# tlkvstepan/PracticalDeepStereo_NIPS2018

Measured on AMD Instinct MI355X. Metric: stereo pairs/sec, 960x540 D=192, Matching+Regularization+SubpixelMap hot path, higher is better.
Workload: dtype f32; 1 GPU; configs[1]: 960x540 pair padded to 576x960, D=192 (48 matching planes, 96 cost planes), batch 1, eval mode, random-init weights seed 0; parallelism=single GPU, launch=eager, whole pairs round-robin over 3 HIP streams

## Files before the change

### practicaldeepstereo_nips2018_amd/csrc/upsample_estimator.hip

```cpp
#include <type_traits>

#include "common.hpp"

namespace pds {

namespace {

constexpr int TR = 4, TC = 32;
constexpr int HR = TR + 2, HC = TC + 2;
constexpr int NPOS = HR * HC;
constexpr int HS = 48;
constexpr int TILE_CH = HR * HS;
constexpr int POS = (NPOS + 63) / 64;
typedef float f32x16 __attribute__((ext_vector_type(16)));
typedef float f32x2 __attribute__((ext_vector_type(2)));

struct FusedArgs {
    const float* __restrict__ in;
    const float* __restrict__ scale;
    const float* __restrict__ shift;
    const float* __restrict__ w;
    const float* __restrict__ bias;
    float* __restrict__ disp;
    float* __restrict__ cost;
    int D, Hi, Wi;
    int lo, hi;
    float step;
    int crop_top, crop_left;
    float* __restrict__ conf;
};

}

constexpr int UHALF = 128;
constexpr int UPOS = (NPOS + UHALF - 1) / UHALF;
constexpr int EO = HC / 2;

template <bool CAND>
__device__ __forceinline__ void estimator_update2(float v, float h1, float h2, int k, int km1, int km2, float& best, int& bi,
                                                  float& bp0, float& bp1, float& bn0, float& bn1) {
    unsigned long long m0, m1, mu;
    if constexpr (CAND) {
        asm volatile(
            "v_cmp_eq_u32_e64 %[m0], %[bi], %[km1]\n\t"
            "v_cmp_eq_u32_e64 %[m1], %[bi], %[km2]\n\t"
            "v_cmp_gt_f32_e64 %[mu], %[v], %[best]\n\t"
            "v_cndmask_b32_e64 %[bn0], %[bn0], %[v], %[m0]\n\t"
            "v_cndmask_b32_e64 %[bn1], %[bn1], %[v], %[m1]\n\t"
            "s_nop 0\n\t"
            "v_cndmask_b32_e64 %[best], %[best], %[v], %[mu]\n\t"
            "v_cndmask_b32_e64 %[bi], %[bi], %[kv], %[mu]\n\t"
            "v_cndmask_b32_e64 %[bp0], %[bp0], %[h1], %[mu]\n\t"
            "v_cndmask_b32_e64 %[bp1], %[bp1], %[h2], %[mu]"
            : [m0] "=&s"(m0), [m1] "=&s"(m1), [mu] "=&s"(mu), [best] "+v"(best), [bi] "+v"(bi), [bp0] "+v"(bp0),
              [bp1] "+v"(bp1), [bn0] "+v"(bn0), [bn1] "+v"(bn1)
            : [v] "v"(v), [h1] "v"(h1), [h2] "v"(h2), [kv] "v"(k), [km1] "s"(km1), [km2] "s"(km2));
    } else {
        asm volatile(
            "v_cmp_eq_u32_e64 %[m0], %[bi], %[km1]\n\t"
            "v_cmp_eq_u32_e64 %[m1], %[bi], %[km2]\n\t"
            "s_nop 1\n\t"
            "v_cndmask_b32_e64 %[bn0], %[bn0], %[v], %[m0]\n\t"
            "v_cndmask_b32_e64 %[bn1], %[bn1], %[v], %[m1]"
            : [m0] "=&s"(m0), [m1] "=&s"(m1), [bn0] "+v"(bn0), [bn1] "+v"(bn1)
            : [v] "v"(v), [bi] "v"(bi), [km1] "s"(km1), [km2] "s"(km2));
    }
}

template <int CIN, int T, bool WRITE_COST, int PY, int DS, bool CONF, bool MIRROR>
__device__ __forceinline__ void upsample_sweep(const FusedArgs& A, float (*tile)[CIN][TILE_CH], float* merge, const int part) {
    constexpr int R = 3 + T;
    constexpr int U = (R % 2 == 0) ? R : 2 * R;
    const int tid = threadIdx.x & (UHALF - 1);
    const int lane = tid & 63;
    const int r = lane >> 4, cp = lane & 15;
    const int i0 = blockIdx.y * TR, j0 = blockIdx.x * TC;
    const int b = blockIdx.z;
    const size_t plane = (size_t)A.Hi * A.Wi;
    const size_t cstride = (size_t)A.D * plane;
    const unsigned plane_bytes = (unsigned)(plane * sizeof(float)), cbytes = (unsigned)(cstride * sizeof(float));
    const __amdgpu_buffer_rsrc_t rsrc = __builtin_amdgcn_make_buffer_rsrc(
        const_cast<float*>(A.in + (size_t)b * CIN * cstride), 0, (int)(CIN * cstride * sizeof(float)), 0x00020000);

    const int per = (A.D + DS - 1) / DS;
    const int lo = DS == 1 ? 0 : part * per, hi = DS == 1 ? A.D : min(A.D, lo + per);
    const int pb = DS == 1 ? 0 : max(lo - T - 1, 0);
    const int pe = WRITE_COST ? A.D : hi + T;
    int nsteps = pe - pb + 1;
    if (DS > 1) {
#pragma unroll
        for (int q = 0; q < DS; ++q) {
            const int lq = q * per, hq = min(A.D, lq + per);
            nsteps = max(nsteps, hq + T - max(lq - T - 1, 0) + 1);
        }
    }

    unsigned goff[UPOS];
    int loff[UPOS];
    bool inside[UPOS];
#pragma unroll
    for (int k = 0; k < UPOS; ++k) {
        const int p = min(tid + k * UHALF, NPOS - 1);
        const int rr = p / HC, cc = p % HC;
        const int y = i0 - 1 + rr, x = j0 - 1 + cc;
        inside[k] = y >= 0 && y < A.Hi && x >= 0 && x < A.Wi;
#ifdef PDS_UPS_NOHALO
        goff[k] = (unsigned)(min(max(y, i0), min(i0 + TR, A.Hi) - 1) * A.Wi + min(max(x, j0), min(j0 + TC, A.Wi) - 1)) * 4u;
#else
        goff[k] = inside[k] ? (unsigned)(y * A.Wi + x) * 4u : 0x80000000u;
#endif
        loff[k] = rr * HS + (cc & 1) * EO + (cc >> 1);
    }
    float sc[CIN], shv[CIN][UPOS];
#pragma unroll
    for (int c = 0; c < CIN; ++c) {
        sc[c] = A.scale ? A.scale[b * CIN + c] : 1.f;
        const float sh = A.scale ? A.shift[b * CIN + c] : 0.f;
#pragma unroll
        for (int k = 0; k < UPOS; ++k) shv[c][k] = inside[k] ? sh : 0.f;
    }
    const float bias = A.bias ? A.bias[0] : 0.f;

    float st[2][CIN][UPOS];
#ifdef PDS_UPS_NOLDSWRITE
    float sink = 0.f;
#define PDS_UPS_STORE(dst_, v_) sink += (v_);
#else
#define PDS_UPS_STORE(dst_, v_) dst_ = (v_);
#endif
#define PDS_FETCHP(set_, p_)                                                       \
    _Pragma("unroll") for (int c = 0; c < CIN; ++c) _Pragma("unroll") for (int k = 0; k < UPOS; ++k) \
        st[set_][c][k] = __builtin_bit_cast(float, __builtin_amdgcn_raw_buffer_load_b32(               \
            rsrc, goff[k], (unsigned)(p_) * plane_bytes + c * cbytes, 0));
#define PDS_STASHP(set_, buf_)                                                     \
    _Pragma("unroll") for (int c = 0; c < CIN; ++c) _Pragma("unroll") for (int k = 0; k < UPOS; ++k) \
        PDS_UPS_STORE(tile[buf_][c][loff[k]], fmaf(sc[c], st[set_][c][k], shv[c][k]))

#ifdef PDS_UPS_TIMING
    long long tm[4] = {0, 0, 0, 0};
#endif
    float best[4], bprev[4][T], bnext[4][T], mass[4];
    int bi[4];
#pragma unroll
    for (int o = 0; o < 4; ++o) {
        best[o] = -INFINITY;
        if constexpr (CONF) mass[o] = 0.f;
        bi[o] = lo;
#pragma unroll
        for (int t = 0; t < T; ++t) bprev[o][t] = bnext[o][t] = -INFINITY;
    }
    f32x2 ring[R][2];
#pragma unroll
    for (int q = 0; q < R; ++q) ring[q][0] = ring[q][1] = f32x2{bias, bias};

    PDS_FETCHP(1, pb)
    if (pb + 1 < A.D) PDS_FETCHP(0, pb + 1)
    PDS_STASHP(1, 0)
    __syncthreads();

    const int lbase = r * HS + cp;
    auto plane_step = [&](auto jc, const int step) __attribute__((always_inline)) {
        constexpr int J = decltype(jc)::value;
        constexpr int SF = J % R, S0 = (J + 1) % R, S1 = (J + 2) % R;
        constexpr int SX = J & 1, SY = SX ^ 1;
        const int p = pb + step;
        ring[S1][0] = ring[S1][1] = f32x2{bias, bias};
#ifdef PDS_UPS_TIMING
        const long long t0 = __builtin_readcyclecounter();
        long long t1 = t0, t2 = t0;
#endif
        if (p < A.D && p <= pe) {
#ifndef PDS_UPS_NOSTAGE
            if (p + 2 < A.D && p + 2 <= pe) PDS_FETCHP(SY, p + 2)
#endif
#pragma nounroll
            for (int c2 = 0; c2 < CIN; c2 += 2) {
                f32x2 r02[2][2], r13[2][2];
#pragma unroll
                for (int cc = 0; cc < 2; ++cc)
#pragma unroll
                    for (int a = 0; a < 2; ++a) {
                        const int vr = (a == 0) ? 1 : (PY == 0 ? 0 : 2);
                        const float* row = &tile[SX][c2 + cc][lbase + vr * HS];
#ifdef PDS_UPS_NOLDSREAD
                        r02[cc][a] = f32x2{sc[cc], shv[a][0]};
                        r13[cc][a] = f32x2{shv[cc][1], sc[a]};
                        continue;
#endif
                        r02[cc][a] = f32x2{row[0], row[1]};
                        r13[cc][a] = f32x2{row[EO], row[EO + 1]};
                    }
                f32x16 wk[3];
#ifdef PDS_UPS_NOSLOAD
// ... 97 lines not shown
                        bprev[o][t] = up ? ring[SP][o >> 1][o & 1] : bprev[o][t];
                    }
                }
            }
        }
#ifdef PDS_UPS_TIMING
        tm[3] += __builtin_readcyclecounter() - t3;
#endif
    };
#ifdef PDS_UPS_TIMING
    const long long t_begin = __builtin_readcyclecounter();
#endif
    for (int base = 0; base < nsteps; base += U) {
#define PDS_STEP(J_) if (base + J_ < nsteps) plane_step(std::integral_constant<int, J_>{}, base + J_);
        PDS_STEP(0) PDS_STEP(1) PDS_STEP(2) PDS_STEP(3)
        if constexpr (U > 4) { PDS_STEP(4) PDS_STEP(5) PDS_STEP(6) PDS_STEP(7) PDS_STEP(8) PDS_STEP(9) }
        if constexpr (U > 10) { PDS_STEP(10) PDS_STEP(11) PDS_STEP(12) PDS_STEP(13) }
#undef PDS_STEP
    }
    static_assert(U == 4 || U == 10 || U == 14, "unrolled groups of T = 1, 2, 4");
#ifdef PDS_UPS_TIMING
    {
        const int wgl = blockIdx.y * gridDim.x + blockIdx.x;
        unsigned hwid, xcc;
        asm volatile("s_getreg_b32 %0, hwreg(HW_REG_HW_ID)" : "=s"(hwid));
        asm volatile("s_getreg_b32 %0, hwreg(HW_REG_XCC_ID)" : "=s"(xcc));
        if (lane == 0 && (wgl % 97) == 0)
            printf("[ups] wg %d part %d py %d xcc %u hwid %08x: start %lld total %lld | channels %lld stash %lld barrier %lld estimator %lld (%d steps)\n",
                   wgl, part, PY, xcc & 15, hwid, t_begin, (long long)__builtin_readcyclecounter() - t_begin, tm[0], tm[1], tm[2], tm[3], nsteps);
    }
#endif
#undef PDS_FETCHP
#undef PDS_STASHP
#undef PDS_UPS_STORE
#ifdef PDS_UPS_NOLDSWRITE
    if (sink == 12345.f) best[0] = sink;
#endif

    if (WRITE_COST) return;
    if (DS > 1) {
        constexpr int ITEMS = 4 * (2 + 2 * T) + (CONF ? 4 : 0);
        float* mine = merge + ((size_t)(part > 0 ? part - 1 : 0) * 2 + PY) * ITEMS * 64 + lane;
        if (part > 0) {
#pragma unroll
            for (int o = 0; o < 4; ++o) {
                mine[(o * (2 + 2 * T) + 0) * 64] = best[o];
                mine[(o * (2 + 2 * T) + 1) * 64] = __int_as_float(bi[o]);
#pragma unroll
                for (int t = 0; t < T; ++t) {
                    mine[(o * (2 + 2 * T) + 2 + t) * 64] = bprev[o][t];
                    mine[(o * (2 + 2 * T) + 2 + T + t) * 64] = bnext[o][t];
                }
                if constexpr (CONF) mine[(4 * (2 + 2 * T) + o) * 64] = mass[o];
            }
        }
        __syncthreads();
        if (part > 0) return;
#pragma unroll
        for (int q = 1; q < DS; ++q) {
            const float* theirs = merge + ((size_t)(q - 1) * 2 + PY) * ITEMS * 64 + lane;
#pragma unroll
            for (int o = 0; o < 4; ++o) {
                const float other = theirs[(o * (2 + 2 * T) + 0) * 64];
                if constexpr (CONF) {
                    const float m = fmaxf(best[o], other);
                    mass[o] = mass[o] * expf(best[o] - m) + theirs[(4 * (2 + 2 * T) + o) * 64] * expf(other - m);
                }
                const bool up = other > best[o];
                best[o] = up ? other : best[o];
                bi[o] = up ? __float_as_int(theirs[(o * (2 + 2 * T) + 1) * 64]) : bi[o];
// ... 48 lines not shown
                float* cdst = A.conf + ((size_t)b * Hc + row) * Wc;
                if (vec) {
                    *reinterpret_cast<float4*>(cdst + mcol) = make_float4(cres[3], cres[2], cres[1], cres[0]);
                } else {
#pragma unroll
                    for (int o = 0; o < 4; ++o)
                        if (o < valid && col + o >= 0) cdst[Wc - 1 - col - o] = cres[o];
                }
            }
        } else if (row >= 0) {
            float* dst = A.disp + ((size_t)b * Hc + row) * Wc + col;
            const int valid = (j + 1 < A.Wi) ? 4 : 2;
            if (valid == 4 && col >= 0 && ((A.crop_left | Wc) & 3) == 0) {
                *reinterpret_cast<float4*>(dst) = make_float4(res[0], res[1], res[2], res[3]);
            } else {
#pragma unroll
                for (int o = 0; o < 4; ++o)
                    if (o < valid && col + o >= 0) dst[o] = res[o];
            }
            if constexpr (CONF) {
                float* cdst = A.conf + ((size_t)b * Hc + row) * Wc + col;
                if (valid == 4 && col >= 0 && ((A.crop_left | Wc) & 3) == 0) {
                    *reinterpret_cast<float4*>(cdst) = make_float4(cres[0], cres[1], cres[2], cres[3]);
                } else {
#pragma unroll
                    for (int o = 0; o < 4; ++o)
                        if (o < valid && col + o >= 0) cdst[o] = cres[o];
                }
            }
        }
    }
}

template <int CIN, int T, bool WRITE_COST, int DS, bool CONF = false, bool MIRROR = false>
__global__ __launch_bounds__(UHALF * DS, (DS == 2 && T <= 2) ? ((CONF && T == 2) ? 4 : 5) : 1) void upsample_full_subpixel_kernel(const FusedArgs A) {
    constexpr int TILE = 2 * CIN * TILE_CH, MERGE = (DS - 1) * 2 * (4 * (2 + 2 * T) + (CONF ? 4 : 0)) * 64;
    constexpr int FLOATS = DS * TILE > MERGE ? DS * TILE : MERGE;
    __shared__ __attribute__((aligned(16))) float lds[FLOATS];
    const int wave = __builtin_amdgcn_readfirstlane(threadIdx.x >> 6);
    const int part = wave >> 1;
    float (*tile)[CIN][TILE_CH] = reinterpret_cast<float (*)[CIN][TILE_CH]>(lds + part * TILE);
    if ((wave & 1) == 0)
        upsample_sweep<CIN, T, WRITE_COST, 0, DS, CONF, MIRROR>(A, tile, lds, part);
    else
        upsample_sweep<CIN, T, WRITE_COST, 1, DS, CONF, MIRROR>(A, tile, lds, part);
}

__global__ void upsample_weight_pairs_kernel(const float* __restrict__ w, float* __restrict__ w_pairs, int cin) {
    const int e = blockIdx.x * blockDim.x + threadIdx.x;
    if (e >= cin * 48) return;
    const int j = e & 3, a = (e >> 2) & 1, kd = (e >> 3) % 3, c = (e / 24) % cin, py = e / (24 * cin);
    const int kh = a == 0 ? 1 + py : 3 - 3 * py;
    w_pairs[e] = w[((c * 3 + kd) * 4 + kh) * 4 + ((j + 1) & 3)];
}

int launch_upsample_weight_pairs(const float* w, float* w_pairs, int cin, hipStream_t s) {
    const int total = cin * 48;
    hipLaunchKernelGGL(upsample_weight_pairs_kernel, dim3((total + 255) / 256), dim3(256), 0, s, w, w_pairs, cin);
    return check_launch("upsample_weight_pairs");
}

bool upsample_estimator_supported(int cin, int lo, int hi) {
    const int t = (-lo > hi) ? -lo : hi;
    return cin == 4 && t >= 1 && t <= 4;
}

int launch_upsample_estimator(const float* in, const float* scale, const float* shift, const float* w,
                              const float* bias, float* disp, int batch, int cin, int d, int hi_, int wi, int lo,
                              int hi, int step, int crop_top, int crop_left, hipStream_t s, float* conf, bool mirror) {
    FusedArgs A;
    A.conf = conf;
    A.crop_top = crop_top;
    A.crop_left = crop_left;
    A.in = in;
    A.scale = scale;
    A.shift = shift;
    A.w = w;
    A.bias = bias;
    A.disp = disp;
    A.D = d;
    A.Hi = hi_;
    A.Wi = wi;
    A.lo = lo;
    A.hi = hi;
    A.step = (float)step;
    dim3 grid((wi + TC - 1) / TC, (hi_ + TR - 1) / TR, batch);
    const int t = (-lo > hi) ? -lo : hi;
    if (cin != 4) return set_error(-1, "upsample_estimator: unsupported channel count %d", cin);
    A.cost = nullptr;
    if (mirror) {
        if (conf) {
            if (t <= 1)
                hipLaunchKernelGGL((upsample_full_subpixel_kernel<4, 1, false, 2, true, true>), grid, dim3(2 * UHALF), 0, s,
                                   A);
            else if (t <= 2)
                hipLaunchKernelGGL((upsample_full_subpixel_kernel<4, 2, false, 2, true, true>), grid, dim3(2 * UHALF), 0, s,
                                   A);
            else
                hipLaunchKernelGGL((upsample_full_subpixel_kernel<4, 4, false, 2, true, true>), grid, dim3(2 * UHALF), 0, s,
                                   A);
            return check_launch("upsample_full_subpixel_confidence_mirrored");
        }
        if (t <= 1)
            hipLaunchKernelGGL((upsample_full_subpixel_kernel<4, 1, false, 2, false, true>), grid, dim3(2 * UHALF), 0, s, A);
        else if (t <= 2)
            hipLaunchKernelGGL((upsample_full_subpixel_kernel<4, 2, false, 2, false, true>), grid, dim3(2 * UHALF), 0, s, A);
        else
            hipLaunchKernelGGL((upsample_full_subpixel_kernel<4, 4, false, 2, false, true>), grid, dim3(2 * UHALF), 0, s, A);
        return check_launch("upsample_full_subpixel_mirrored");
    }
    if (conf) {
        if (t <= 1)
            hipLaunchKernelGGL((upsample_full_subpixel_kernel<4, 1, false, 2, true>), grid, dim3(2 * UHALF), 0, s, A);
        else if (t <= 2)
            hipLaunchKernelGGL((upsample_full_subpixel_kernel<4, 2, false, 2, true>), grid, dim3(2 * UHALF), 0, s, A);
        else
            hipLaunchKernelGGL((upsample_full_subpixel_kernel<4, 4, false, 2, true>), grid, dim3(2 * UHALF), 0, s, A);
        return check_launch("upsample_full_subpixel_confidence");
    }
    if (t <= 1)
        hipLaunchKernelGGL((upsample_full_subpixel_kernel<4, 1, false, 2>), grid, dim3(2 * UHALF), 0, s, A);
    else if (t <= 2)
        hipLaunchKernelGGL((upsample_full_subpixel_kernel<4, 2, false, 2>), grid, dim3(2 * UHALF), 0, s, A);
    else
        hipLaunchKernelGGL((upsample_full_subpixel_kernel<4, 4, false, 2>), grid, dim3(2 * UHALF), 0, s, A);
    return check_launch("upsample_full_subpixel");
}

bool upsample_full_valu_supported(int cin) { return cin == 4; }

int launch_upsample_full(const float* in, const float* scale, const float* shift, const float* w, const float* bias,
                         float* cost, int batch, int cin, int d, int hi_, int wi, hipStream_t s) {
    if (cin != 4) return set_error(-1, "upsample_full: unsupported channel count %d", cin);
    FusedArgs A;
    A.in = in;
    A.scale = scale;
    A.shift = shift;
    A.w = w;
    A.bias = bias;
    A.disp = nullptr;
    A.cost = cost;
    A.D = d;
    A.Hi = hi_;
    A.Wi = wi;
    A.lo = 0;
    A.hi = 0;
    A.step = 0.f;
    A.crop_top = A.crop_left = 0;
    A.conf = nullptr;
    dim3 grid((wi + TC - 1) / TC, (hi_ + TR - 1) / TR, batch);
    hipLaunchKernelGGL((upsample_full_subpixel_kernel<4, 1, true, 1>), grid, dim3(UHALF), 0, s, A);
    return check_launch("upsample_full");
}

}
```

### practicaldeepstereo_nips2018_amd/csrc/conv2d_t8.hip

```cpp
#include <atomic>
#include <type_traits>

#include "common.hpp"

namespace pds {

namespace {

constexpr int C2_THREADS = 256;
constexpr int C2_CIN = 64, C2_COUT = 8, C2_KC = 4, C2_CHUNKS = C2_CIN / C2_KC;
constexpr int C2_TY = 16, C2_NB = 2, C2_TX = 16 * C2_NB, C2_RP = C2_TY / 8;
constexpr int C2_YT = C2_TY + 2, C2_XT = C2_TX + 2, C2_RS = 36;
constexpr int C2_PART = C2_YT * C2_RS * 8;
constexpr int C2_BUF = 2 * C2_PART;
constexpr int C2_AFRAGS = C2_CHUNKS * 3 * 2;
constexpr int C2_ABYTES = C2_AFRAGS * 64 * 8;
constexpr int C2_NPOS = C2_YT * C2_XT;
constexpr int C2_POS = (C2_NPOS + C2_THREADS - 1) / C2_THREADS;
static_assert(C2_RS >= C2_XT, "LDS row");
typedef float f32x4 __attribute__((ext_vector_type(4)));
typedef _Float16 f16x4 __attribute__((ext_vector_type(4)));

struct C2Args {
    Src a, b;
// ... 279 lines not shown
        if (c == C2_CHUNKS - 1) {
            const int out_base = (int)((size_t)Pcur.nb * C2_COUT * cstride * sizeof(float));
#pragma unroll
            for (int p = 0; p < C2_RP; ++p)
#pragma unroll
                for (int r = 0; r < 4; ++r) {
                    const int h = r >> 1, y = Pcur.y0 + 2 * (C2_RP * wave + p) + (r & 1);
                    const int row_bytes = __builtin_amdgcn_readfirstlane(
                        out_base + (int)(((size_t)Pcur.d * A.H + min(y, A.H - 1)) * A.W + Pcur.x0) * (int)sizeof(float));
#pragma unroll
                    for (int j = 0; j < C2_NB; ++j) {
                        float t = acc[p][j][r] * SC.unscale;
                        if (A.lrelu) t = fmaxf(t, t * kLeakySlope);
                        const bool ok = y < A.H && Pcur.x0 + 16 * j + n16 < A.W;
                        __builtin_amdgcn_raw_buffer_store_b32(__builtin_bit_cast(int, t), ro,
                                                              ok ? out_lane + (h ? out_c1 : 0u) + 64u * j : ~0u, row_bytes, 0);
                    }
                }
        }
        __syncthreads();
    };
    for (int g = 0; g < total_chunks; g += 4) {
        step(g, S1(), S0());
        step(g + 1, S2(), S1());
        step(g + 2, S3(), S2());
        step(g + 3, S0(), S3());
    }
}

constexpr int C2W_THREADS = 512;
constexpr int C2W_MAXW = 352;
typedef unsigned u32x4 __attribute__((ext_vector_type(4)));

template <bool TWO, int NBH, int C2W_TY, int C2W_ITEMS>
__global__ __launch_bounds__(C2W_THREADS, 2) void conv2d_t8w_kernel(const C2Args A) {
    constexpr int C2W_YT = C2W_TY + 2;
    extern __shared__ __attribute__((aligned(16))) unsigned char lds[];
    unsigned char* abuf = lds;
    unsigned char* ibuf = lds + C2_ABYTES;
    const int RSW = A.W + 4, QW = A.W >> 2;
    const int part_bytes = C2W_YT * RSW * 8, buf_bytes = 2 * part_bytes;

    const int tid = threadIdx.x;
    const int lane = tid & 63;
    const int wave = __builtin_amdgcn_readfirstlane(tid >> 6);
    const int pair = wave & 3, half = wave >> 2;
    const int n16 = lane & 15, q = lane >> 4;
    const size_t plane = (size_t)A.H * A.W;
    const size_t cstride = (size_t)A.D * plane;
    const int cbytes = (int)(cstride * sizeof(float));
    const __amdgpu_buffer_rsrc_t ra = __builtin_amdgcn_make_buffer_rsrc(
        const_cast<float*>(A.a.p), 0, (int)((size_t)A.N * C2_CIN * cstride * sizeof(float)), 0x00020000);
    const __amdgpu_buffer_rsrc_t rb = __builtin_amdgcn_make_buffer_rsrc(
        const_cast<float*>(TWO ? A.b.p : A.a.p), 0, (int)((size_t)A.N * C2_CIN * cstride * sizeof(float)), 0x00020000);
    const __amdgpu_buffer_rsrc_t ro = __builtin_amdgcn_make_buffer_rsrc(
        A.out, 0, (int)((size_t)A.N * C2_COUT * cstride * sizeof(float)), 0x00020000);

    const C2Scales SC = c2_scales(A, TWO, reinterpret_cast<float*>(ibuf));
    for (int e = tid; e < C2_CHUNKS * 3 * 64; e += C2W_THREADS) {
        const int l = e & 63, f = e >> 6;
        const int m = l & 15, oc = m >> 1, py = m & 1, yi = l >> 4, dy = yi - py;
        const int chunk = f / 3, dx = f % 3;
        float wv[4];
#pragma unroll
        for (int i = 0; i < 4; ++i)
            wv[i] = (dy >= 0 && dy <= 2)
                        ? A.w[((size_t)oc * C2_CIN + chunk * C2_KC + i) * 9 + dy * 3 + dx] * SC.ws
                        : 0.f;
        f16x4 hi, lo;
        c2_split(wv, hi, lo);
        *reinterpret_cast<f16x4*>(abuf + ((size_t)(f * 2 + 0) * 64 + l) * 8) = hi;
        *reinterpret_cast<f16x4*>(abuf + ((size_t)(f * 2 + 1) * 64 + l) * 8) = lo;
    }
    for (int e = tid; e < 2 * 2 * C2W_YT * 2; e += C2W_THREADS) {
        const int side = e & 1, row = e >> 1;
        *reinterpret_cast<unsigned long long*>(ibuf + ((size_t)row * RSW + (side ? A.W + 2 : 1)) * 8) = 0ull;
    }

    const int xcd = blockIdx.x & 7, slot = blockIdx.x >> 3, per_xcd = gridDim.x >> 3;
// ... 80 lines not shown
            cs[ch] = vs[SET][ch] * SC.as;
            chs[ch] = vh[SET][ch] * SC.as;
        }
#pragma unroll
        for (int k = 0; k < C2W_ITEMS; ++k)
#pragma unroll
            for (int pp = 0; pp < 2; ++pp) {
                f16x8 hi2, lo2;
#pragma unroll
                for (int e = 0; e < 2; ++e) {
                    const int px = 2 * pp + e;
                    float v[4];
#pragma unroll
                    for (int ch = 0; ch < C2_KC; ++ch) {
                        float t = cs[ch] * va[SET][k][ch][px];
                        if (TWO) t = fmaf(SC.as, vb[SET][k][ch][px], t);
                        v[ch] = fmaf(chs[ch], inside_regs[SET][k], t);
                    }
                    f16x4 hi, lo;
                    c2_split(v, hi, lo);
#pragma unroll
                    for (int i = 0; i < 4; ++i) {
                        hi2[4 * e + i] = hi[i];
                        lo2[4 * e + i] = lo[i];
                    }
                }
                *reinterpret_cast<f16x8*>(buf + lo_off[k] + pp * lo_step[k]) = hi2;
                *reinterpret_cast<f16x8*>(buf + part_bytes + lo_off[k] + pp * lo_step[k]) = lo2;
            }
    };

    const float bscale = SC.ws * SC.as;
    const float bias0 = (A.bias ? A.bias[2 * q] : 0.f) * bscale, bias1 = (A.bias ? A.bias[2 * q + 1] : 0.f) * bscale;
    const int b_base = ((2 * pair + q) * RSW + 16 * half * NBH + n16 + 1) * 8;
    const unsigned out_lane = (unsigned)((size_t)(2 * q) * cstride + 16 * half * NBH + n16) * 4u;
    const unsigned out_c1 = (unsigned)cstride * 4u;

    using S0 = std::integral_constant<int, 0>;
    using S1 = std::integral_constant<int, 1>;
    int fetched_tile = -1;
    auto fetch_chunk = [&](int g, auto set_c) {
        const int gf = min(g, total_chunks - 1);
        if (gf / C2_CHUNKS != fetched_tile) {
            fetched_tile = gf / C2_CHUNKS;
            prepare(fetched_tile, goff, inside, sbase, gidx);
        }
        fetch(gf, set_c);
    };
    __syncthreads();
    if (total_chunks > 0) {
        fetch_chunk(0, S0());
        stash(ibuf, S0());
        fetch_chunk(1, S1());
        fetch_chunk(2, S0());
    }
    __syncthreads();

    f32x4 acc[NBH];
    TilePos Pcur = tile_pos(0);
#ifdef PDS_C2W_TIMING
    long long tmw[5] = {0, 0, 0, 0, 0};
#endif
    auto step = [&](int g, auto set_c) {
        const int c = g % C2_CHUNKS;
        if (c == 0) {
            Pcur = tile_pos(g / C2_CHUNKS);
#pragma unroll
            for (int j = 0; j < NBH; ++j) acc[j] = f32x4{bias0, bias0, bias1, bias1};
        }
        const int gf = min(g + 3, total_chunks - 1);
        const bool new_tile = gf / C2_CHUNKS != fetched_tile;
        if (new_tile) prepare(gf / C2_CHUNKS, goff_n, inside_n, sbase_n, gidx_n);
        fetched_tile = gf / C2_CHUNKS;

        const unsigned char* buf = ibuf + (g & 1) * buf_bytes + b_base;
#ifdef PDS_C2W_TIMING
        const long long tt0 = __builtin_readcyclecounter();
#endif
        stash(ibuf + ((g + 1) & 1) * buf_bytes, set_c);
#ifdef PDS_C2W_TIMING
        asm volatile("s_waitcnt lgkmcnt(0)" ::: "memory");
        const long long tt1 = __builtin_readcyclecounter();
#endif
#pragma unroll
        for (int k = 0; k < C2W_ITEMS; ++k) {
            inside[k] = new_tile ? inside_n[k] : inside[k];
            goff[k] = new_tile ? goff_n[k] : goff[k];
        }
        sbase = new_tile ? sbase_n : sbase;
        gidx = new_tile ? gidx_n : gidx;
        fetch(gf, set_c);
#ifdef PDS_C2W_TIMING
        const long long tt2 = __builtin_readcyclecounter();
#endif
        const unsigned char* af = abuf + ((size_t)c * 3 * 2 * 64 + lane) * 8;
#pragma unroll
        for (int dx = 0; dx < 3; ++dx) {
            const f16x4 a_hi = *reinterpret_cast<const f16x4*>(af + (dx * 2 + 0) * 512);
            const f16x4 a_lo = *reinterpret_cast<const f16x4*>(af + (dx * 2 + 1) * 512);
#pragma unroll
            for (int j = 0; j < NBH; ++j) {
                const unsigned char* bp = buf + (16 * j + dx) * 8;
                const f16x4 b_hi = *reinterpret_cast<const f16x4*>(bp);
                const f16x4 b_lo = *reinterpret_cast<const f16x4*>(bp + part_bytes);
                acc[j] = __builtin_amdgcn_mfma_f32_16x16x16f16(a_hi, b_lo, acc[j], 0, 0, 0);
                acc[j] = __builtin_amdgcn_mfma_f32_16x16x16f16(a_lo, b_hi, acc[j], 0, 0, 0);
                acc[j] = __builtin_amdgcn_mfma_f32_16x16x16f16(a_hi, b_hi, acc[j], 0, 0, 0);
            }
        }
#ifndef PDS_C2W_TIMING
#pragma unroll
        for (int i = 0; i < 3 * NBH * 3; ++i) {
            __builtin_amdgcn_sched_group_barrier(0x008, 1, 0);
            __builtin_amdgcn_sched_group_barrier(0x100, 1, 0);
            __builtin_amdgcn_sched_group_barrier(0x002, 4, 0);
            __builtin_amdgcn_sched_group_barrier(0x200, 1, 0);
            __builtin_amdgcn_sched_group_barrier(0x020, 1, 0);
        }
#else
        const long long tt3 = __builtin_readcyclecounter();
        tmw[0] += tt1 - tt0; tmw[1] += tt2 - tt1; tmw[2] += tt3 - tt2;
#endif
        if (c == C2_CHUNKS - 1) {
            const int out_base = (int)((size_t)Pcur.nb * C2_COUT * cstride * sizeof(float));
#pragma unroll
            for (int r = 0; r < 4; ++r) {
                const int h = r >> 1, y = Pcur.y0 + 2 * pair + (r & 1);
                const int row_bytes = __builtin_amdgcn_readfirstlane(
                    out_base + (int)(((size_t)Pcur.d * A.H + min(y, A.H - 1)) * A.W) * (int)sizeof(float));
#pragma unroll
                for (int j = 0; j < NBH; ++j) {
                    float t = acc[j][r] * SC.unscale;
                    if (A.lrelu) t = fmaxf(t, t * kLeakySlope);
                    const bool ok = 2 * pair < C2W_TY && y < A.H && 16 * (half * NBH + j) + n16 < A.W;
                    __builtin_amdgcn_raw_buffer_store_b32(__builtin_bit_cast(int, t), ro,
                                                          ok ? out_lane + (h ? out_c1 : 0u) + 64u * j : ~0u, row_bytes, 0);
                }
            }
        }
#ifdef PDS_C2W_TIMING
        const long long tt4 = __builtin_readcyclecounter();
#endif
        __syncthreads();
#ifdef PDS_C2W_TIMING
        tmw[3] += __builtin_readcyclecounter() - tt4;
        tmw[4] += 1;
#endif
    };
#ifdef PDS_C2W_TIMING
    const long long t_all = __builtin_readcyclecounter();
#endif
    for (int g = 0; g < total_chunks; g += 2) {
        step(g, S1());
        step(g + 1, S0());
    }
#ifdef PDS_C2W_TIMING
    if (lane == 0 && (blockIdx.x % 61) == 0 && (wave == 0 || wave == 5))
        printf("[t8w] wg %d wave %d: total %lld | stash(+wait) %lld fetch-issue %lld mfma %lld barrier %lld over %lld chunks (%d tiles)\n",
               (int)blockIdx.x, wave, (long long)__builtin_readcyclecounter() - t_all, tmw[0], tmw[1], tmw[2], tmw[3], tmw[4], my_tiles);
#endif
}

namespace {

bool c2t8_enabled() {
    static const bool on = []() {
        const char* e = debug_switch("PDS_CONV2D_T8");
        return !(e && e[0] == '0');
    }();
    return on;
}

template <bool TWO, bool NA, bool NB2>
int launch_c2t8(const C2Args& A, hipStream_t s) {
    constexpr size_t lds_bytes = (size_t)C2_ABYTES + 2 * C2_BUF;
    static std::atomic<unsigned> attr_done{0};
    if (DeviceOnce once{attr_done}) {
        (void)hipFuncSetAttribute(reinterpret_cast<const void*>(&conv2d_t8_kernel<TWO, NA, NB2>),
                                  hipFuncAttributeMaxDynamicSharedMemorySize, (int)(160 * 1024));
    }
    int wgs = 512;
    if (wgs > A.tiles) wgs = (A.tiles + 7) / 8 * 8;
    hipLaunchKernelGGL((conv2d_t8_kernel<TWO, NA, NB2>), dim3(wgs), dim3(C2_THREADS), lds_bytes, s, A);
    return check_launch("conv2d_t8");
}

}

bool c2t8_wide(const ConvLayer& L) {
    static const bool on = []() {
        const char* e = debug_switch("PDS_CONV2D_T8W");
        return !(e && e[0] == '0');
    }();
    if (!on) return false;
    if (!L.a.scale || (L.b.p && L.b.scale)) return false;
    return (L.in.w & 3) == 0 && L.in.w >= 64 && L.in.w <= C2W_MAXW && L.in.h >= 8;
}

template <bool TWO, int NBH, int TY, int ITEMS>
int launch_c2t8w(C2Args& A, hipStream_t s) {
    A.tiles_x = 1;
    A.tiles_y = (A.H + TY - 1) / TY;
    A.tiles = A.N * A.D * A.tiles_y;
    const size_t lds_bytes = (size_t)C2_ABYTES + 2 * 2 * (size_t)(TY + 2) * (A.W + 4) * 8 + 2 * (size_t)(A.W + 4) * 8 + 256;
    static std::atomic<unsigned> attr_done{0};
    static int cus[32] = {0};
    int dev = 0;
    (void)hipGetDevice(&dev);
    if (DeviceOnce once{attr_done}) {
        (void)hipFuncSetAttribute(reinterpret_cast<const void*>(&conv2d_t8w_kernel<TWO, NBH, TY, ITEMS>),
                                  hipFuncAttributeMaxDynamicSharedMemorySize, (int)(160 * 1024));
        int n = 0;
        (void)hipDeviceGetAttribute(&n, hipDeviceAttributeMultiprocessorCount, dev);
        cus[dev & 31] = n > 0 ? n : 256;
    }
    int wgs = cus[dev & 31] / 8 * 8;
    if (wgs > A.tiles) wgs = (A.tiles + 7) / 8 * 8;
    const int probe = probe_before("conv2d_t8w", s);
    hipLaunchKernelGGL((conv2d_t8w_kernel<TWO, NBH, TY, ITEMS>), dim3(wgs), dim3(C2W_THREADS), lds_bytes, s, A);
    probe_after(probe, A.tiles, s);
    return check_launch("conv2d_t8w");
}

int c2t8w_rows(int w) {
    static const int forced = []() {
        const char* e = debug_switch("PDS_CONV2D_T8W_ROWS");
        return e ? atoi(e) : 0;
    }();
    if (forced == 8 || forced == 6) return forced;
    return 8 * (w >> 2) <= C2W_THREADS ? 6 : 8;
}

bool conv2d_t8_supported(const ConvLayer& L) {
    if (!c2t8_enabled()) return false;
    if (L.kd != 1 || L.stride != 1 || L.in.c != C2_CIN || L.out_g.c != C2_COUT) return false;
    if (L.l0A || L.side_out || L.plane_weight_sets > 0) return false;
    if (!L.a.bounded) return false;
    if (L.b.p && !L.b.bounded) return false;
    if (L.b.p && L.b.bcast_d) return false;
    if ((size_t)L.in.n * C2_CIN * L.in.d * L.in.h * L.in.w >= ((size_t)1 << 29)) return false;
    const long tiles = (long)L.in.n * L.in.d * ((L.in.h + C2_TY - 1) / C2_TY) * ((L.in.w + C2_TX - 1) / C2_TX);
    return tiles < (1L << 30);
}

int launch_conv2d_t8(const ConvLayer& L, hipStream_t s) {
    C2Args A;
    A.a = L.a;
    A.b = L.b;
    A.w = L.weight;
    A.bias = L.bias;
    A.out = L.out;
    A.N = L.in.n;
    A.D = L.in.d;
    A.H = L.in.h;
    A.W = L.in.w;
    A.lrelu = L.lrelu;
    A.tiles_x = (A.W + C2_TX - 1) / C2_TX;
    A.tiles_y = (A.H + C2_TY - 1) / C2_TY;
    A.tiles = A.N * A.D * A.tiles_y * A.tiles_x;
    if (!A.a.bound || A.a.bound_n <= 0 || (L.b.p && (!A.b.bound || A.b.bound_n <= 0)))
        return set_error(-1, "conv2d_t8: a source without a range bound");
    if (c2t8_wide(L)) {
        const int blocks = (A.W + 15) / 16, nbh = (blocks + 1) / 2;
        const int rows = c2t8w_rows(A.W), items = ((rows + 2) * (A.W >> 2) + C2W_THREADS - 1) / C2W_THREADS;
        if (nbh <= 8 && rows == 6 && items == 1)
            return L.b.p ? launch_c2t8w<true, 8, 6, 1>(A, s) : launch_c2t8w<false, 8, 6, 1>(A, s);
        if (nbh <= 8) return L.b.p ? launch_c2t8w<true, 8, 8, 2>(A, s) : launch_c2t8w<false, 8, 8, 2>(A, s);
        return L.b.p ? launch_c2t8w<true, 11, 8, 2>(A, s) : launch_c2t8w<false, 11, 8, 2>(A, s);
    }
    const bool na = L.a.scale != nullptr, nb2 = L.b.p && L.b.scale;
    if (L.b.p) {
        if (na) return nb2 ? launch_c2t8<true, true, true>(A, s) : launch_c2t8<true, true, false>(A, s);
        return nb2 ? launch_c2t8<true, false, true>(A, s) : launch_c2t8<true, false, false>(A, s);
    }
    return na ? launch_c2t8<false, true, false>(A, s) : launch_c2t8<false, false, false>(A, s);
}

}
```

Measured before the change: 441.4 pairs/s.

## Stage upsample halo tiles with 128-bit quad loads split by channel per wave

Adds a WIDE staging path to the fused upsample/subpixel sweep. Each lane issues one 128-bit buffer load covering four adjacent columns of one channel, and the two waves in a pair stage alternating channels, instead of every thread issuing scalar 32-bit loads for all channels. The even/odd-split LDS layout gets extra padding and a one-element shift so the deinterleaved quads can be written as two 8-byte stores. The intent is fewer global load and LDS store instructions per plane. A scalar fallback stays for unaligned inputs or widths not divisible by four, with a lower occupancy bound for that path, and the debug-only timing and no-write macros are removed.

After: 442.7 pairs/s, median of 5. About the same (+0.3%).

```diff
diff --git a/practicaldeepstereo_nips2018_amd/csrc/upsample_estimator.hip b/practicaldeepstereo_nips2018_amd/csrc/upsample_estimator.hip
--- a/practicaldeepstereo_nips2018_amd/csrc/upsample_estimator.hip
+++ b/practicaldeepstereo_nips2018_amd/csrc/upsample_estimator.hip
@@ -14,6 +14,7 @@
 constexpr int POS = (NPOS + 63) / 64;
 typedef float f32x16 __attribute__((ext_vector_type(16)));
 typedef float f32x2 __attribute__((ext_vector_type(2)));
+typedef float f32x4 __attribute__((ext_vector_type(4)));
 
 struct FusedArgs {
     const float* __restrict__ in;
@@ -34,7 +35,7 @@
 
 constexpr int UHALF = 128;
 constexpr int UPOS = (NPOS + UHALF - 1) / UHALF;
-constexpr int EO = HC / 2;
+constexpr int EO = HC / 2 + 2;
 
 template <bool CAND>
 __device__ __forceinline__ void estimator_update2(float v, float h1, float h2, int k, int km1, int km2, float& best, int& bi,
@@ -67,7 +68,7 @@
     }
 }
 
-template <int CIN, int T, bool WRITE_COST, int PY, int DS, bool CONF, bool MIRROR>
+template <int CIN, int T, bool WRITE_COST, int PY, int DS, bool CONF, bool MIRROR, bool WIDE>
 __device__ __forceinline__ void upsample_sweep(const FusedArgs& A, float (*tile)[CIN][TILE_CH], float* merge, const int part) {
     constexpr int R = 3 + T;
     constexpr int U = (R % 2 == 0) ? R : 2 * R;
@@ -95,46 +96,73 @@
         }
     }
 
+    constexpr int QROW = (TC + 8) / 4, QCH = QROW * HR;
+    static_assert(QCH <= 64 && CIN == 2 * UPOS, "slot k of wave PY stages channel 2 k + PY");
+    constexpr int NST = WIDE ? 4 : CIN;
+    constexpr int NSC = WIDE ? 1 : CIN;
     unsigned goff[UPOS];
     int loff[UPOS];
-    bool inside[UPOS];
-#pragma unroll
-    for (int k = 0; k < UPOS; ++k) {
-        const int p = min(tid + k * UHALF, NPOS - 1);
-        const int rr = p / HC, cc = p % HC;
-        const int y = i0 - 1 + rr, x = j0 - 1 + cc;
-        inside[k] = y >= 0 && y < A.Hi && x >= 0 && x < A.Wi;
-#ifdef PDS_UPS_NOHALO
-        goff[k] = (unsigned)(min(max(y, i0), min(i0 + TR, A.Hi) - 1) * A.Wi + min(max(x, j0), min(j0 + TC, A.Wi) - 1)) * 4u;
-#else
-        goff[k] = inside[k] ? (unsigned)(y * A.Wi + x) * 4u : 0x80000000u;
-#endif
-        loff[k] = rr * HS + (cc & 1) * EO + (cc >> 1);
-    }
-    float sc[CIN], shv[CIN][UPOS];
-#pragma unroll
-    for (int c = 0; c < CIN; ++c) {
-        sc[c] = A.scale ? A.scale[b * CIN + c] : 1.f;
-        const float sh = A.scale ? A.shift[b * CIN + c] : 0.f;
-#pragma unroll
-        for (int k = 0; k < UPOS; ++k) shv[c][k] = inside[k] ? sh : 0.f;
+    float scv[NSC][UPOS], shv[NSC][UPOS];
+    if constexpr (WIDE) {
+        const int q = min(lane, QCH - 1), chi = PY;
+        const int rr = q / QROW, qi = q % QROW;
+        const int y = i0 - 1 + rr, x = j0 - 4 + 4 * qi;
+        const bool inside = y >= 0 && y < A.Hi && x >= 0 && x < A.Wi;
+#pragma unroll
+        for (int k = 0; k < UPOS; ++k) {
+            const int c = 2 * k + chi;
+            goff[k] = inside ? (unsigned)(y * A.Wi + x) * 4u : 0x80000000u;
+            loff[k] = c * TILE_CH + rr * HS + 2 * qi;
+            scv[0][k] = A.scale ? A.scale[b * CIN + c] : 1.f;
+            shv[0][k] = inside && A.scale ? A.shift[b * CIN + c] : 0.f;
+        }
+    } else {
+#pragma unroll
+        for (int k = 0; k < UPOS; ++k) {
+            const int p = min(tid + k * UHALF, NPOS - 1);
+            const int rr = p / HC, cc = p % HC;
+            const int y = i0 - 1 + rr, x = j0 - 1 + cc;
+            const bool inside = y >= 0 && y < A.Hi && x >= 0 && x < A.Wi;
+            goff[k] = inside ? (unsigned)(y * A.Wi + x) * 4u : 0x80000000u;
+            loff[k] = rr * HS + (cc & 1) * EO + (cc >> 1) + 1;
+#pragma unroll
+            for (int c = 0; c < CIN; ++c) {
+                scv[c][k] = A.scale ? A.scale[b * CIN + c] : 1.f;
+                shv[c][k] = inside && A.scale ? A.shift[b * CIN + c] : 0.f;
+            }
+        }
     }
     const float bias = A.bias ? A.bias[0] : 0.f;
 
-    float st[2][CIN][UPOS];
-#ifdef PDS_UPS_NOLDSWRITE
-    float sink = 0.f;
-#define PDS_UPS_STORE(dst_, v_) sink += (v_);
-#else
-#define PDS_UPS_STORE(dst_, v_) dst_ = (v_);
-#endif
-#define PDS_FETCHP(set_, p_)                                                       \
-    _Pragma("unroll") for (int c = 0; c < CIN; ++c) _Pragma("unroll") for (int k = 0; k < UPOS; ++k) \
-        st[set_][c][k] = __builtin_bit_cast(float, __builtin_amdgcn_raw_buffer_load_b32(               \
-            rsrc, goff[k], (unsigned)(p_) * plane_bytes + c * cbytes, 0));
-#define PDS_STASHP(set_, buf_)                                                     \
-    _Pragma("unroll") for (int c = 0; c < CIN; ++c) _Pragma("unroll") for (int k = 0; k < UPOS; ++k) \
-        PDS_UPS_STORE(tile[buf_][c][loff[k]], fmaf(sc[c], st[set_][c][k], shv[c][k]))
+    float st[2][WIDE ? 1 : CIN][UPOS];
+    f32x4 stq[2][UPOS];
+#define PDS_FETCHP(set_, p_)                                                                                       \
+    {if constexpr (WIDE) {                                                                                         \
+        _Pragma("unroll") for (int k = 0; k < UPOS; ++k) {                                                         \
+            stq[set_][k] = __builtin_bit_cast(f32x4, __builtin_amdgcn_raw_buffer_load_b128(                       \
+                rsrc, goff[k], (unsigned)(p_) * plane_bytes + (2 * k + PY) * cbytes, 0));                          \
+        }                                                                                                          \
+    } else {                                                                                                       \
+        _Pragma("unroll") for (int c = 0; c < CIN; ++c) _Pragma("unroll") for (int k = 0; k < UPOS; ++k)           \
+            st[set_][c][k] = __builtin_bit_cast(float, __builtin_amdgcn_raw_buffer_load_b32(                      \
+                rsrc, goff[k], (unsigned)(p_) * plane_bytes + c * cbytes, 0));                                     \
+    }}
+#define PDS_STASHP(set_, buf_)                                                                                     \
+    {if constexpr (WIDE) {                                                                                         \
+        _Pragma("unroll") for (int k = 0; k < UPOS; ++k) {                                                         \
+            float* dst = &tile[buf_][0][0] + loff[k];                                                              \
+             \
+            asm volatile("" : "+v"(stq[set_][k]));                                                                 \
+            const f32x4 q4 = stq[set_][k];                                                                         \
+            const float v0 = fmaf(scv[0][k], q4[0], shv[0][k]), v1 = fmaf(scv[0][k], q4[1], shv[0][k]),            \
+                        v2 = fmaf(scv[0][k], q4[2], shv[0][k]), v3 = fmaf(scv[0][k], q4[3], shv[0][k]);            \
+            *reinterpret_cast<f32x2*>(dst) = f32x2{v1, v3};                                   \
+            *reinterpret_cast<f32x2*>(dst + EO - 1) = f32x2{v0, v2};                      \
+        }                                                                                                          \
+    } else {                                                                                                       \
+        _Pragma("unroll") for (int c = 0; c < CIN; ++c) _Pragma("unroll") for (int k = 0; k < UPOS; ++k)           \
+            tile[buf_][c][loff[k]] = fmaf(scv[c][k], st[set_][c][k], shv[c][k]);                                   \
+    }}
 
 #ifdef PDS_UPS_TIMING
     long long tm[4] = {0, 0, 0, 0};
@@ -158,7 +186,7 @@
     PDS_STASHP(1, 0)
     __syncthreads();
 
-    const int lbase = r * HS + cp;
+    const int lbase = r * HS + cp + 1;
     auto plane_step = [&](auto jc, const int step) __attribute__((always_inline)) {
         constexpr int J = decltype(jc)::value;
         constexpr int SF = J % R, S0 = (J + 1) % R, S1 = (J + 2) % R;
@@ -322,10 +350,6 @@
 #endif
 #undef PDS_FETCHP
 #undef PDS_STASHP
-#undef PDS_UPS_STORE
-#ifdef PDS_UPS_NOLDSWRITE
-    if (sink == 12345.f) best[0] = sink;
-#endif
 
     if (WRITE_COST) return;
     if (DS > 1) {
@@ -440,8 +464,8 @@
     }
 }
 
-template <int CIN, int T, bool WRITE_COST, int DS, bool CONF = false, bool MIRROR = false>
-__global__ __launch_bounds__(UHALF * DS, (DS == 2 && T <= 2) ? ((CONF && T == 2) ? 4 : 5) : 1) void upsample_full_subpixel_kernel(const FusedArgs A) {
+template <int CIN, int T, bool WRITE_COST, int DS, bool CONF = false, bool MIRROR = false, bool WIDE = true>
+__global__ __launch_bounds__(UHALF * DS, (DS == 2 && T <= 2) ? (((CONF && T == 2) || !WIDE) ? 4 : 5) : 1) void upsample_full_subpixel_kernel(const FusedArgs A) {
     constexpr int TILE = 2 * CIN * TILE_CH, MERGE = (DS - 1) * 2 * (4 * (2 + 2 * T) + (CONF ? 4 : 0)) * 64;
     constexpr int FLOATS = DS * TILE > MERGE ? DS * TILE : MERGE;
     __shared__ __attribute__((aligned(16))) float lds[FLOATS];
@@ -449,9 +473,9 @@
     const int part = wave >> 1;
     float (*tile)[CIN][TILE_CH] = reinterpret_cast<float (*)[CIN][TILE_CH]>(lds + part * TILE);
     if ((wave & 1) == 0)
-        upsample_sweep<CIN, T, WRITE_COST, 0, DS, CONF, MIRROR>(A, tile, lds, part);
+        upsample_sweep<CIN, T, WRITE_COST, 0, DS, CONF, MIRROR, WIDE>(A, tile, lds, part);
     else
-        upsample_sweep<CIN, T, WRITE_COST, 1, DS, CONF, MIRROR>(A, tile, lds, part);
+        upsample_sweep<CIN, T, WRITE_COST, 1, DS, CONF, MIRROR, WIDE>(A, tile, lds, part);
 }
 
 __global__ void upsample_weight_pairs_kernel(const float* __restrict__ w, float* __restrict__ w_pairs, int cin) {
@@ -471,6 +495,34 @@
 bool upsample_estimator_supported(int cin, int lo, int hi) {
     const int t = (-lo > hi) ? -lo : hi;
     return cin == 4 && t >= 1 && t <= 4;
+}
+
+namespace {
+
+bool quads_apply(const float* in, int wi) {
+#ifdef PDS_UPS_NARROW
+    return false;
+#endif
+    return wi % 4 == 0 && reinterpret_cast<uintptr_t>(in) % 16 == 0;
+}
+
+template <bool CONF, bool MIRROR>
+void launch_fused_window(int t, bool wide, dim3 grid, hipStream_t s, const FusedArgs& A) {
+#define PDS_LAUNCH_T(T_)                                                                                                  \
+    if (wide)                                                                                                             \
+        hipLaunchKernelGGL((upsample_full_subpixel_kernel<4, T_, false, 2, CONF, MIRROR, true>), grid, dim3(2 * UHALF), 0, s, A); \
+    else                                                                                                                  \
+        hipLaunchKernelGGL((upsample_full_subpixel_kernel<4, T_, false, 2, CONF, MIRROR, false>), grid, dim3(2 * UHALF), 0, s, A);
+    if (t <= 1) {
+        PDS_LAUNCH_T(1)
+    } else if (t <= 2) {
+        PDS_LAUNCH_T(2)
+    } else {
+        PDS_LAUNCH_T(4)
+    }
+#undef PDS_LAUNCH_T
+}
+
 }
 
 int launch_upsample_estimator(const float* in, const float* scale, const float* shift, const float* w,
@@ -496,42 +548,20 @@
     const int t = (-lo > hi) ? -lo : hi;
     if (cin != 4) return set_error(-1, "upsample_estimator: unsupported channel count %d", cin);
     A.cost = nullptr;
+    const bool wide = quads_apply(in, wi);
     if (mirror) {
         if (conf) {
-            if (t <= 1)
-                hipLaunchKernelGGL((upsample_full_subpixel_kernel<4, 1, false, 2, true, true>), grid, dim3(2 * UHALF), 0, s,
-                                   A);
-            else if (t <= 2)
-                hipLaunchKernelGGL((upsample_full_subpixel_kernel<4, 2, false, 2, true, true>), grid, dim3(2 * UHALF), 0, s,
-                                   A);
-            else
-                hipLaunchKernelGGL((upsample_full_subpixel_kernel<4, 4, false, 2, true, true>), grid, dim3(2 * UHALF), 0, s,
-                                   A);
+            launch_fused_window<true, true>(t, wide, grid, s, A);
             return check_launch("upsample_full_subpixel_confidence_mirrored");
         }
-        if (t <= 1)
-            hipLaunchKernelGGL((upsample_full_subpixel_kernel<4, 1, false, 2, false, true>), grid, dim3(2 * UHALF), 0, s, A);
-        else if (t <= 2)
-            hipLaunchKernelGGL((upsample_full_subpixel_kernel<4, 2, false, 2, false, true>), grid, dim3(2 * UHALF), 0, s, A);
-        else
-            hipLaunchKernelGGL((upsample_full_subpixel_kernel<4, 4, false, 2, false, true>), grid, dim3(2 * UHALF), 0, s, A);
+        launch_fused_window<false, true>(t, wide, grid, s, A);
         return check_launch("upsample_full_subpixel_mirrored");
     }
     if (conf) {
-        if (t <= 1)
-            hipLaunchKernelGGL((upsample_full_subpixel_kernel<4, 1, false, 2, true>), grid, dim3(2 * UHALF), 0, s, A);
-        else if (t <= 2)
-            hipLaunchKernelGGL((upsample_full_subpixel_kernel<4, 2, false, 2, true>), grid, dim3(2 * UHALF), 0, s, A);
-        else
-            hipLaunchKernelGGL((upsample_full_subpixel_kernel<4, 4, false, 2, true>), grid, dim3(2 * UHALF), 0, s, A);
+        launch_fused_window<true, false>(t, wide, grid, s, A);
         return check_launch("upsample_full_subpixel_confidence");
     }
-    if (t <= 1)
-        hipLaunchKernelGGL((upsample_full_subpixel_kernel<4, 1, false, 2>), grid, dim3(2 * UHALF), 0, s, A);
-    else if (t <= 2)
-        hipLaunchKernelGGL((upsample_full_subpixel_kernel<4, 2, false, 2>), grid, dim3(2 * UHALF), 0, s, A);
-    else
-        hipLaunchKernelGGL((upsample_full_subpixel_kernel<4, 4, false, 2>), grid, dim3(2 * UHALF), 0, s, A);
+    launch_fused_window<false, false>(t, wide, grid, s, A);
     return check_launch("upsample_full_subpixel");
 }
 
@@ -557,7 +587,10 @@
     A.crop_top = A.crop_left = 0;
     A.conf = nullptr;
     dim3 grid((wi + TC - 1) / TC, (hi_ + TR - 1) / TR, batch);
-    hipLaunchKernelGGL((upsample_full_subpixel_kernel<4, 1, true, 1>), grid, dim3(UHALF), 0, s, A);
+    if (quads_apply(in, wi))
+        hipLaunchKernelGGL((upsample_full_subpixel_kernel<4, 1, true, 1, false, false, true>), grid, dim3(UHALF), 0, s, A);
+    else
+        hipLaunchKernelGGL((upsample_full_subpixel_kernel<4, 1, true, 1, false, false, false>), grid, dim3(UHALF), 0, s, A);
     return check_launch("upsample_full");
 }
 
```

## Balance wide conv2d_t8 waves by splitting row-pair/block units evenly

Applied to the files above, without the earlier changes.

For the 6-row tile variant, the wide 64->8 conv kernel now splits all (row-pair, 16-column block) work units evenly across the 8 waves instead of a fixed pair/half mapping that left two waves idle. Each wave now holds 6 accumulators instead of 8, with per-unit LDS offsets and output rows; a run may span two row pairs. This is meant to raise MFMA utilisation per workgroup. It adds per-unit address arithmetic and divergent-looking store addressing.

Result: no change. 430.0 pairs/s before, 433.3 pairs/s after (median of 6 runs) (+0.8%).

```diff
diff --git a/practicaldeepstereo_nips2018_amd/csrc/conv2d_t8.hip b/practicaldeepstereo_nips2018_amd/csrc/conv2d_t8.hip
--- a/practicaldeepstereo_nips2018_amd/csrc/conv2d_t8.hip
+++ b/practicaldeepstereo_nips2018_amd/csrc/conv2d_t8.hip
@@ -335,7 +335,30 @@
 constexpr int C2W_MAXW = 352;
 typedef unsigned u32x4 __attribute__((ext_vector_type(4)));
 
-template <bool TWO, int NBH, int C2W_TY, int C2W_ITEMS>
+struct C2WRun {
+    int pair0, blk0, n0, len;
+};
+template <int TY, int NACC>
+__device__ __forceinline__ C2WRun c2w_run(int wave, int blocks) {
+    C2WRun R;
+    if (TY == 8) {
+        R.pair0 = wave & 3;
+        R.blk0 = (wave >> 2) * NACC;
+        R.len = R.n0 = NACC;
+        return R;
+    } else {
+        const int units = (TY / 2) * blocks, base = units >> 3, rem = units & 7;
+        const int u0 = wave * base + min(wave, rem);
+        R.len = min(base + (wave < rem ? 1 : 0), NACC);
+        R.pair0 = u0 / blocks;
+        R.blk0 = u0 - R.pair0 * blocks;
+        R.n0 = min(R.len, blocks - R.blk0);
+    }
+    if (R.len == 0) R.pair0 = R.blk0 = 0;
+    return R;
+}
+
+template <bool TWO, int NACC, int C2W_TY, int C2W_ITEMS>
 __global__ __launch_bounds__(C2W_THREADS, 2) void conv2d_t8w_kernel(const C2Args A) {
     constexpr int C2W_YT = C2W_TY + 2;
     extern __shared__ __attribute__((aligned(16))) unsigned char lds[];
@@ -347,7 +370,7 @@
     const int tid = threadIdx.x;
     const int lane = tid & 63;
     const int wave = __builtin_amdgcn_readfirstlane(tid >> 6);
-    const int pair = wave & 3, half = wave >> 2;
+    const C2WRun R = c2w_run<C2W_TY, NACC>(wave, (A.W + 15) >> 4);
     const int n16 = lane & 15, q = lane >> 4;
     const size_t plane = (size_t)A.H * A.W;
     const size_t cstride = (size_t)A.D * plane;
@@ -494,8 +517,19 @@
 
     const float bscale = SC.ws * SC.as;
     const float bias0 = (A.bias ? A.bias[2 * q] : 0.f) * bscale, bias1 = (A.bias ? A.bias[2 * q + 1] : 0.f) * bscale;
-    const int b_base = ((2 * pair + q) * RSW + 16 * half * NBH + n16 + 1) * 8;
-    const unsigned out_lane = (unsigned)((size_t)(2 * q) * cstride + 16 * half * NBH + n16) * 4u;
+    constexpr bool RUNS = C2W_TY != 8;
+    const int pair = R.pair0, half = wave >> 2;
+    int unit_off[NACC], unit_blk[NACC];
+    bool unit_first[NACC];
+#pragma unroll
+    for (int j = 0; j < NACC; ++j) {
+        const bool used = j < R.len;
+        unit_first[j] = j < R.n0 || !used;
+        unit_blk[j] = !used ? R.blk0 : unit_first[j] ? R.blk0 + j : j - R.n0;
+        unit_off[j] = (2 * (R.pair0 + (unit_first[j] ? 0 : 1)) * RSW + 16 * unit_blk[j]) * 8;
+    }
+    const int b_base = RUNS ? (q * RSW + n16 + 1) * 8 : ((2 * pair + q) * RSW + 16 * half * NACC + n16 + 1) * 8;
+    const unsigned out_lane = (unsigned)((size_t)(2 * q) * cstride + (RUNS ? 0 : 16 * half * NACC) + n16) * 4u;
     const unsigned out_c1 = (unsigned)cstride * 4u;
 
     using S0 = std::integral_constant<int, 0>;
@@ -518,7 +552,7 @@
     }
     __syncthreads();
 
-    f32x4 acc[NBH];
+    f32x4 acc[NACC];
     TilePos Pcur = tile_pos(0);
 #ifdef PDS_C2W_TIMING
     long long tmw[5] = {0, 0, 0, 0, 0};
@@ -528,7 +562,7 @@
         if (c == 0) {
             Pcur = tile_pos(g / C2_CHUNKS);
 #pragma unroll
-            for (int j = 0; j < NBH; ++j) acc[j] = f32x4{bias0, bias0, bias1, bias1};
+            for (int j = 0; j < NACC; ++j) acc[j] = f32x4{bias0, bias0, bias1, bias1};
         }
         const int gf = min(g + 3, total_chunks - 1);
         const bool new_tile = gf / C2_CHUNKS != fetched_tile;
@@ -561,8 +595,8 @@
             const f16x4 a_hi = *reinterpret_cast<const f16x4*>(af + (dx * 2 + 0) * 512);
             const f16x4 a_lo = *reinterpret_cast<const f16x4*>(af + (dx * 2 + 1) * 512);
 #pragma unroll
-            for (int j = 0; j < NBH; ++j) {
-                const unsigned char* bp = buf + (16 * j + dx) * 8;
+            for (int j = 0; j < NACC; ++j) {
+                const unsigned char* bp = buf + (RUNS ? unit_off[j] + dx * 8 : (16 * j + dx) * 8);
                 const f16x4 b_hi = *reinterpret_cast<const f16x4*>(bp);
                 const f16x4 b_lo = *reinterpret_cast<const f16x4*>(bp + part_bytes);
                 acc[j] = __builtin_amdgcn_mfma_f32_16x16x16f16(a_hi, b_lo, acc[j], 0, 0, 0);
@@ -572,7 +606,7 @@
         }
 #ifndef PDS_C2W_TIMING
 #pragma unroll
-        for (int i = 0; i < 3 * NBH * 3; ++i) {
+        for (int i = 0; i < 3 * NACC * 3; ++i) {
             __builtin_amdgcn_sched_group_barrier(0x008, 1, 0);
             __builtin_amdgcn_sched_group_barrier(0x100, 1, 0);
             __builtin_amdgcn_sched_group_barrier(0x002, 4, 0);
@@ -587,16 +621,26 @@
             const int out_base = (int)((size_t)Pcur.nb * C2_COUT * cstride * sizeof(float));
 #pragma unroll
             for (int r = 0; r < 4; ++r) {
-                const int h = r >> 1, y = Pcur.y0 + 2 * pair + (r & 1);
-                const int row_bytes = __builtin_amdgcn_readfirstlane(
-                    out_base + (int)(((size_t)Pcur.d * A.H + min(y, A.H - 1)) * A.W) * (int)sizeof(float));
-#pragma unroll
-                for (int j = 0; j < NBH; ++j) {
+                const int h = r >> 1, y0 = Pcur.y0 + 2 * pair + (r & 1);
+                const int row_bytes0 = __builtin_amdgcn_readfirstlane(
+                    out_base + (int)(((size_t)Pcur.d * A.H + min(y0, A.H - 1)) * A.W) * (int)sizeof(float));
+                const int row_bytes1 = __builtin_amdgcn_readfirstlane(
+                    out_base + (int)(((size_t)Pcur.d * A.H + min(y0 + 2, A.H - 1)) * A.W) * (int)sizeof(float));
+#pragma unroll
+                for (int j = 0; j < NACC; ++j) {
                     float t = acc[j][r] * SC.unscale;
                     if (A.lrelu) t = fmaxf(t, t * kLeakySlope);
-                    const bool ok = 2 * pair < C2W_TY && y < A.H && 16 * (half * NBH + j) + n16 < A.W;
-                    __builtin_amdgcn_raw_buffer_store_b32(__builtin_bit_cast(int, t), ro,
-                                                          ok ? out_lane + (h ? out_c1 : 0u) + 64u * j : ~0u, row_bytes, 0);
+                    if (RUNS) {
+                        const int y = unit_first[j] ? y0 : y0 + 2;
+                        const bool ok = j < R.len && y < A.H && 16 * unit_blk[j] + n16 < A.W;
+                        __builtin_amdgcn_raw_buffer_store_b32(__builtin_bit_cast(int, t), ro,
+                                                              ok ? out_lane + (h ? out_c1 : 0u) : ~0u,
+                                                              (unit_first[j] ? row_bytes0 : row_bytes1) + 64 * unit_blk[j], 0);
+                    } else {
+                        const bool ok = y0 < A.H && 16 * (half * NACC + j) + n16 < A.W;
+                        __builtin_amdgcn_raw_buffer_store_b32(__builtin_bit_cast(int, t), ro,
+                                                              ok ? out_lane + (h ? out_c1 : 0u) + 64u * j : ~0u, row_bytes0, 0);
+                    }
                 }
             }
         }
@@ -659,7 +703,7 @@
     return (L.in.w & 3) == 0 && L.in.w >= 64 && L.in.w <= C2W_MAXW && L.in.h >= 8;
 }
 
-template <bool TWO, int NBH, int TY, int ITEMS>
+template <bool TWO, int NACC, int TY, int ITEMS>
 int launch_c2t8w(C2Args& A, hipStream_t s) {
     A.tiles_x = 1;
     A.tiles_y = (A.H + TY - 1) / TY;
@@ -670,7 +714,7 @@
     int dev = 0;
     (void)hipGetDevice(&dev);
     if (DeviceOnce once{attr_done}) {
-        (void)hipFuncSetAttribute(reinterpret_cast<const void*>(&conv2d_t8w_kernel<TWO, NBH, TY, ITEMS>),
+        (void)hipFuncSetAttribute(reinterpret_cast<const void*>(&conv2d_t8w_kernel<TWO, NACC, TY, ITEMS>),
                                   hipFuncAttributeMaxDynamicSharedMemorySize, (int)(160 * 1024));
         int n = 0;
         (void)hipDeviceGetAttribute(&n, hipDeviceAttributeMultiprocessorCount, dev);
@@ -679,7 +723,7 @@
     int wgs = cus[dev & 31] / 8 * 8;
     if (wgs > A.tiles) wgs = (A.tiles + 7) / 8 * 8;
     const int probe = probe_before("conv2d_t8w", s);
-    hipLaunchKernelGGL((conv2d_t8w_kernel<TWO, NBH, TY, ITEMS>), dim3(wgs), dim3(C2W_THREADS), lds_bytes, s, A);
+    hipLaunchKernelGGL((conv2d_t8w_kernel<TWO, NACC, TY, ITEMS>), dim3(wgs), dim3(C2W_THREADS), lds_bytes, s, A);
     probe_after(probe, A.tiles, s);
     return check_launch("conv2d_t8w");
 }
@@ -726,7 +770,7 @@
         const int blocks = (A.W + 15) / 16, nbh = (blocks + 1) / 2;
         const int rows = c2t8w_rows(A.W), items = ((rows + 2) * (A.W >> 2) + C2W_THREADS - 1) / C2W_THREADS;
         if (nbh <= 8 && rows == 6 && items == 1)
-            return L.b.p ? launch_c2t8w<true, 8, 6, 1>(A, s) : launch_c2t8w<false, 8, 6, 1>(A, s);
+            return L.b.p ? launch_c2t8w<true, 6, 6, 1>(A, s) : launch_c2t8w<false, 6, 6, 1>(A, s);
         if (nbh <= 8) return L.b.p ? launch_c2t8w<true, 8, 8, 2>(A, s) : launch_c2t8w<false, 8, 8, 2>(A, s);
         return L.b.p ? launch_c2t8w<true, 11, 8, 2>(A, s) : launch_c2t8w<false, 11, 8, 2>(A, s);
     }
```
